# anzeA/Tarok

Measured on AMD Instinct MI355X. Metric: env steps/sec at 65 536 parallel 4-player games; 1/2/4/8 MI355X, higher is better.
Workload: dtype u64

## Files before the change

include/tarok_env.h:

```cpp
#ifndef TAROK_ENV_H
#define TAROK_ENV_H
#include <stdint.h>

#ifdef __cplusplus
extern "C" {
#endif

#define TAROK_ABI_VERSION 5
#define TAROK_MAX_CARDS_PER_LAUNCH 192
#define TAROK_GAMES_AHEAD 14

#define TAROK_OK 0
#define TAROK_EINVAL (-1)
#define TAROK_EHIP (-2)
#define TAROK_ENOMEM (-3)
#define TAROK_ENODEV (-4)

#define TAROK_MIX_ALL 0
#define TAROK_MIX_NAVADNA3 1
#define TAROK_MIX_BOT 2
#define TAROK_MIX_FIXED 16

#define TAROK_DEFER_EXCHANGE 1
#define TAROK_AUTO_RESET 2
// ... 7 lines not shown
#define TAROK_OBS_DONE (1ULL << 62)
#define TAROK_OBS_ERROR (1ULL << 63)

#define TAROK_LANE_HAND0 0
#define TAROK_LANE_PILE0 4
#define TAROK_LANE_TALON 8
#define TAROK_LANE_META 9
#define TAROK_NUM_LANES 10

typedef struct tarok_env tarok_env;

const char *tarok_strerror(int code);
int tarok_abi_version(void);
int tarok_device_count(void);
int tarok_last_hip_error(void);

int tarok_create(tarok_env **out, int device, int64_t n_games, uint64_t game_offset,
                 uint64_t seed, int mix, int flags);
void tarok_destroy(tarok_env *env);
int64_t tarok_num_games(const tarok_env *env);

#define TAROK_OPT_REFILL_FAN 2
#define TAROK_OPT_LAZY_REFILL 3
int tarok_set_option(tarok_env *env, int option, int value);

int tarok_reset(tarok_env *env, uint32_t episode, const uint8_t *deals, const int8_t *contract,
                const int8_t *declarer, const int8_t *king_suit, const int8_t *talon_choice,
                const uint8_t *discards, int flags, void *stream);

int tarok_exchange(tarok_env *env, const int8_t *talon_choice, const uint8_t *discards, void *stream);

int tarok_legal_actions(tarok_env *env, uint64_t *obs_out, int8_t *seat_out, void *stream);

int tarok_step(tarok_env *env, const uint8_t *action, int16_t *reward_out, uint8_t *done_out,
               uint16_t *trick_out, uint64_t *obs_out, int flags, void *stream);

int tarok_prefetch(tarok_env *env, void *stream);

int tarok_policy_random(tarok_env *env, const uint64_t *obs, uint8_t *action_out, void *stream);

int tarok_step_random(tarok_env *env, uint8_t *action_out, int16_t *reward_out, uint8_t *done_out,
                      uint16_t *trick_out, uint64_t *obs_out, int flags, void *stream);

int tarok_krog_random(tarok_env *env, int cards, int64_t stride, uint8_t *action_out, int16_t *reward_out,
                      uint8_t *done_out, uint16_t *trick_out, uint64_t *obs_out, int flags, void *stream);

// ... 109 lines not shown
```

tarok_amd/csrc/tarok_env.hip:

```cpp
#include "tarok_device.h"

#include <hip/hip_runtime.h>
#include <stdint.h>
#include <stdio.h>
#include <stdlib.h>
#include <string.h>
#include <type_traits>
#include <utility>

#include "../../include/tarok_env.h"

#define TK_BLOCK 256
#define TK_PF_SLOTS (4 * TK_BLOCK)
#define TK_GRAPH_CACHE 16
#define TK_REFILL_CAP (TK_BLOCK * TK_AHEAD)
#define TK_REFILL_FAN 8
#define TK_RC(group, k) ((((size_t)(group)) * 4 + (k)) * 32)
#define TK_BULK_EVERY 32u
#define TK_BULK_CAP ((TK_BULK_EVERY / 4) * TK_BLOCK)

#define TK_AHEAD TAROK_GAMES_AHEAD
#define TK_LINE(episode) ((u32)(episode) % (u32)TK_AHEAD)
#define TK_FINQ 128
#define TK_STREAM_STORE(ptr, val) __builtin_nontemporal_store((val), (ptr))
#define TK_WAIT_LOADS() __builtin_amdgcn_s_waitcnt(0x0F70)
#define TK_RARE(c) __builtin_expect(!!(c), 0)
#define TK_USUAL(c) __builtin_expect(!!(c), 1)

struct __attribute__((aligned(64))) AuxLine {
    ulonglong2 n01, n23; u64 nkey; u32 nep;
    u32 pad[5];
};
struct __attribute__((aligned(64))) Aux { AuxLine line[TK_AHEAD]; };
static_assert(sizeof(AuxLine) == 64 && sizeof(Aux) == 64 * TK_AHEAD, "64 bytes per next-game line");
static_assert((TK_BLOCK * sizeof(Aux)) % 128 == 0, "a play group's next-game lines end on an L2 line boundary");
static_assert(TK_AHEAD >= 2 && TK_AHEAD <= 15, "epar / cprev are 4-bit fields");
struct __attribute__((aligned(32))) Counters {
    int4 score_sum;
    u32 episode;
    u32 pad[3];
};
static_assert(sizeof(Counters) == 32, "Counters is half a cache line");

struct tarok_env {
    int device;
    int64_t n;
    u64 offset, seed;
    int mix, flags;
    ulonglong2 *s01, *s23;
    Aux *aux;
    Counters *cnt;
    uint16_t *nstale;
    u64 *gkey;
    uint8_t *hist;
    u64 *rlist;
    u32 *rcount;
    u64 *elist;
    u32 *epoch;
    uint32_t refill_fan;
    uint32_t lazy_refill;
    int n_cus;
    float *adam_sumsq;
    u64 *stamps;
    size_t stamps_words;
    int launched;
    hipStream_t cap_stream;
    struct GraphEntry {
        hipGraphExec_t exec;
        int fused, chunk, flags, prefetch;
        void *action, *reward, *done, *obs, *stamps;
        uint32_t fan, lazy;
    } graphs[TK_GRAPH_CACHE];
    int n_graphs;
};

static thread_local int g_last_hip = 0;

#define HIPCHK(x)                                                   \
    do {                                                            \
        hipError_t e_ = (x);                                        \
        if (e_ != hipSuccess) { g_last_hip = (int)e_; return TAROK_EHIP; } \
    } while (0)

static inline dim3 grid_for(int64_t n) { return dim3((unsigned)((n + TK_BLOCK - 1) / TK_BLOCK)); }

__device__ __forceinline__ void load_game(Game &g, const ulonglong2 *s01, const ulonglong2 *s23, int64_t i) {
    ulonglong2 a = s01[i], b = s23[i];
    unpack(g, a.x, a.y, b.x, b.y);
}
__device__ __forceinline__ void store_game(const Game &g, ulonglong2 *s01, ulonglong2 *s23, int64_t i,
                                           bool seats_changed = true) {
    ulonglong2 a;
    pack_play(g, a.x, a.y);
// ... 253 lines not shown
            for (u32 q = 0; q < TK_REFILL_FAN; q++) {
                bool has = q < fan && g0 + q < play_groups;
                cum[q + 1] = cum[q] + (has ? min(tk_ld(&rcount[TK_RC(g0 + q, 2 + which)]), (u32)TK_BULK_CAP) : 0u);
            }
        }
        for (u32 j = tid; j < cum[TK_REFILL_FAN]; j += nthreads) {
            u32 q = 0;
#pragma unroll
            for (u32 r = 1; r < TK_REFILL_FAN; r++) q += j >= cum[r] ? 1u : 0u;
            u32 base = 0;
#pragma unroll
            for (u32 r = 0; r < TK_REFILL_FAN; r++) base = (r == q) ? cum[r] : base;
            u64 en = tk_ld(&lists[((int64_t)(g0 + q) * 2 + which) * cap + (j - base)]);
            deal_into_buffer(aux, (int64_t)(g0 + q) * TK_BLOCK + (u32)(en & 0xFFFF), (u32)(en >> 32), seed, offset, mix);
        }
    }
    if (any || bulk) {
        __syncthreads();
        if (any && tid < fan && g0 + tid < play_groups) rcount[TK_RC(g0 + tid, par ^ 1u)] = 0u;
        if (bulk && tid < fan && g0 + tid < play_groups) rcount[TK_RC(g0 + tid, 2 + which)] = 0u;
    }
}

template <bool HIST>
__device__ __forceinline__ void play_role(
    u32 group, u32 tid,
    int64_t n, u64 seed, u64 offset, int mix, int flags, int cards, int64_t stride, TkCount count, u32 *epoch, u32 play_groups, u32 fan,
    uint8_t *__restrict__ action_out, int16_t *__restrict__ reward,
    uint8_t *__restrict__ done, uint16_t *__restrict__ trick, u64 *__restrict__ obs, uint8_t *__restrict__ hist,
    ulonglong2 *__restrict__ s01, ulonglong2 *__restrict__ s23, Aux *aux, Counters *__restrict__ cnt,
    u64 *__restrict__ gkey, u64 *rlist, u32 *rcount, u64 *__restrict__ stamps) {
    __shared__ unsigned short push_list[TK_REFILL_CAP];
    __shared__ u32 push_ep[TK_BLOCK];
    __shared__ u32 push_count;
    __shared__ u32 finq[TK_BLOCK / 64][9][TK_FINQ];
    __shared__ int sacc[4][TK_BLOCK];
    if (tid == 0) push_count = 0;
    sacc[0][tid] = 0; sacc[1][tid] = 0; sacc[2][tid] = 0; sacc[3][tid] = 0;
    __syncthreads();
    u32 fq_head = 0, fq_n = 0;
    u32 (*fq)[TK_FINQ] = finq[tid >> 6];
    auto drain_finished = [&](u32 cnt_) __attribute__((always_inline)) {
        u32 lane = tid & 63;
        if (lane < cnt_) {
            u32 e = (fq_head + lane) & (TK_FINQ - 1);
            Game f;
            f.A = TK_U64(fq[0][e], fq[1][e]); f.B = TK_U64(fq[2][e], fq[3][e]); f.C = TK_U64(fq[4][e], fq[5][e]);
            u32 m = fq[7][e], ri = fq[8][e];
            f.talon = TK_U64(fq[6][e], (m >> 24) & 15u);
            f.contract = m & 15; f.declarer = (m >> 4) & 3; f.king = (m >> 6) & 3; f.team = (m >> 8) & 15;
            f.tl = (m >> 12) & 7; f.trick_no = (m >> 16) & 15; f.leader = (m >> 20) & 3;
            f.trick = 0; f.nt = 0; f.phase = TK_PHASE_DONE; f.error = 0; f.epar = 0; f.cprev = 0;
            u64 sc = final_scores(f);
            u32 t = ri & 0xFFFFu;
            if (reward) {
                u64 rs = sc;
                if ((flags & TAROK_REWARD_REF) && (f.contract == TK_BERAC || f.contract == TK_ODPRTI_BERAC)) {
                    int dv = f.trick_no >= 12 ? -20 : 20;
                    u32 d = f.declarer;
                    rs = pack_scores(d == 0 ? (int)(int16_t)(sc & 0xFFFF) : dv, d == 1 ? (int)(int16_t)((sc >> 16) & 0xFFFF) : dv,
                                     d == 2 ? (int)(int16_t)((sc >> 32) & 0xFFFF) : dv, d == 3 ? (int)(int16_t)(sc >> 48) : dv);
                }
                reinterpret_cast<u64 *>(reward)[(int64_t)group * TK_BLOCK + t + (int64_t)(ri >> 16) * stride] = rs;
            }
            atomicAdd(&sacc[0][t], (int)(int16_t)(sc & 0xFFFF)); atomicAdd(&sacc[1][t], (int)(int16_t)((sc >> 16) & 0xFFFF));
            atomicAdd(&sacc[2][t], (int)(int16_t)((sc >> 32) & 0xFFFF)); atomicAdd(&sacc[3][t], (int)(int16_t)(sc >> 48));
        }
        fq_head = (fq_head + cnt_) & (TK_FINQ - 1);
        fq_n -= cnt_;
    };
    u64 t_real0 = 0, t_cyc0 = 0, t_play = 0;
    if (stamps) { t_real0 = __builtin_amdgcn_s_memrealtime(); t_cyc0 = __builtin_amdgcn_s_memtime(); }
    int64_t i = (int64_t)group * TK_BLOCK + tid;
    bool valid = i < n;
    int64_t ic = valid ? i : n - 1;
    Game g;
    load_game(g, s01, s23, ic);
    u64 key = gkey[ic];
    bool autoreset = (flags & TAROK_AUTO_RESET) != 0;
    bool berac = g.contract == TK_BERAC || g.contract == TK_ODPRTI_BERAC;
    bool spec = valid && ((g.phase == TK_PHASE_PLAY && (int)g.nt + cards >= 4 &&
                           (berac || (int)(g.trick_no * 4 + g.nt) + cards >= 48)) ||
                          g.phase == TK_PHASE_DONE);
    u32 cprev0 = valid ? g.cprev : 0u;
    u32 allowed = TK_AHEAD - min(cprev0, (u32)TK_AHEAD);
    int4 acc = make_int4(0, 0, 0, 0);
    u32 cur_ep = 0;
    ulonglong2 na = make_ulonglong2(0, 0), nb = na, na2 = na, nb2 = na;
    u64 nkey = 0, nkey2 = 0;
    u32 nep1 = 0, nep2 = 0;
    bool ok1 = false, ok2 = false;
    auto line_tag = [&](bool &ok, u32 &nep, u32 tag) __attribute__((always_inline)) { nep = tag; ok = true; };
// ... 22 lines not shown
    u64 legal = (valid && g.phase == TK_PHASE_PLAY) ? legal_now(g) : 0;
    u64 c_lead = 0;
    u64 pending = 0;
    u32 blocked_v = 0, resync_v = 0;
    auto fetch_lines = [&](bool lacks, bool lacks2) __attribute__((always_inline)) {
        if (lacks) {
            const AuxLine *ln = &aux[i].line[TK_LINE(cur_ep + 1)];
            na = ln->n01; nb = ln->n23; nkey = ln->nkey;
            line_tag(ok1, nep1, ln->nep);
        }
        if (lacks2) {
            const AuxLine *l2 = &aux[i].line[TK_LINE(cur_ep + 2)];
            na2 = l2->n01; nb2 = l2->n23; nkey2 = l2->nkey;
            line_tag(ok2, nep2, l2->nep);
        }
    };
    auto play_card = [&](auto all_tag, auto nt_tag, auto std_tag, int64_t row, int ci) __attribute__((always_inline)) {
        constexpr bool ALL = decltype(all_tag)::value;
        constexpr int NT = decltype(nt_tag)::value;
        constexpr bool STD = decltype(std_tag)::value;
        if constexpr (NT >= 0) g.nt = (u32)NT;
        constexpr bool TOP_UP_EARLY = ALL && NT == 0;
        constexpr bool TOP_UP_LATE = !(ALL && NT == 3);
        if constexpr (TOP_UP_EARLY) {
            if (TK_RARE(pending != 0)) {
                pending = 0;
                bool base = spec && blocked_v == 0 && consumed >= 1;
                bool lacks = base && nep1 != cur_ep + 1 && consumed < allowed;
                bool lacks2 = base && nep2 != cur_ep + 2 && consumed + 1 < allowed;
                fetch_lines(lacks, lacks2);
            }
        }
        const bool v = ALL ? true : valid;
        const bool play = ALL ? true : (valid && g.phase == TK_PHASE_PLAY);
        u32 a = play ? policy_action(key, g.trick_no * 4 + g.nt, legal) : 255u;
        u64 scores = 0;
        u32 trick_info = 0;
        int res = -2;
        const u32 pos = g.trick_no * 4 + g.nt;
        if constexpr (ALL && NT == 0) c_lead = g.C;
        const u64 *lead_plane = (ALL && NT >= 0) ? &c_lead : nullptr;
        if (play) res = apply_step<true, true>(g, a, scores, trick_info, !STD && trick != nullptr, lead_plane);
        bool fin = res == 1;
        if (HIST && hist && play && res >= 0) hist[(int64_t)pos * n + i] = (uint8_t)a;
        if constexpr (!(ALL && NT >= 0)) {
            touched = touched || res != -2;
            seats_dirty = seats_dirty || (res >= 0 && g.nt == 0);
        }
        if (v) {
            if (STD || action_out) TK_STREAM_STORE(&action_out[row], (uint8_t)a);
            if (!STD && trick) TK_STREAM_STORE(&trick[row], (uint16_t)trick_info);
        }
        constexpr bool CAN_END = !(ALL && NT >= 0 && NT < 3);
        constexpr bool FAST_RENEW = ALL && NT == 3;
        auto push_finished = [&](u64 fm, u32 slot0) __attribute__((always_inline)) {
            u32 e = (slot0 + __builtin_amdgcn_mbcnt_hi((u32)(fm >> 32), __builtin_amdgcn_mbcnt_lo((u32)fm, 0))) & (TK_FINQ - 1);
            fq[0][e] = TK_LO(g.A); fq[1][e] = TK_HI(g.A); fq[2][e] = TK_LO(g.B); fq[3][e] = TK_HI(g.B);
            fq[4][e] = TK_LO(g.C); fq[5][e] = TK_HI(g.C); fq[6][e] = TK_LO(g.talon);
            u32 m = (g.declarer << 4) | g.contract;      TK_KEEP_VGPR(m);
            m = (g.king << 6) | m;                       TK_KEEP_VGPR(m);
            m = (g.team << 8) | m;                       TK_KEEP_VGPR(m);
            m = (g.tl << 12) | m;                        TK_KEEP_VGPR(m);
            m = (g.trick_no << 16) | m;                  TK_KEEP_VGPR(m);
            m = (g.leader << 20) | m;                    TK_KEEP_VGPR(m);
            fq[7][e] = (TK_HI(g.talon) << 24) | m;
            fq[8][e] = ((u32)ci << 16) | tid;
        };
        auto swap_in = [&]() __attribute__((always_inline)) {
            unpack_fresh(g, na.x, na.y, nb.x, nb.y);
            key = nkey;
            na = na2; nb = nb2; nkey = nkey2;
            nep1 = nep2;
        };
        auto deal_in_place = [&](bool deal_here, Game &gd, u64 &kd) __attribute__((always_inline)) {
            u64 pend = __ballot(deal_here);
            if (TK_RARE(pend != 0)) {
                u64 dkey = 0;
                if (deal_here) dkey = game_key(seed, offset + (u64)i, cur_ep + 1);
                u64 h0 = 0, h1 = 0, h2 = 0, h3 = 0, tal = 0;
                u32 lane = __lane_id();
                while (pend) {
                    int l = __builtin_ctzll(pend);
                    pend &= pend - 1;
                    u32 klo = (u32)__builtin_amdgcn_readlane((int)(u32)dkey, l);
                    u32 khi = (u32)__builtin_amdgcn_readlane((int)(u32)(dkey >> 32), l);
                    u64 w0, w1, w2, w3, wt;
                    deal_wave(klo, khi, w0, w1, w2, w3, wt);
                    if (lane == (u32)l) { h0 = w0; h1 = w1; h2 = w2; h3 = w3; tal = wt; }
                }
                if (deal_here) {
                    u32 cc, d, k;
                    sample_setup(dkey, mix, cc, d, k);
                    setup_game(gd, h0, h1, h2, h3, tal, cc, d, k);
                    gd.epar = TK_LINE(cur_ep + 1); gd.cprev = 0;
                    if (gd.phase == TK_PHASE_EXCHANGE) bot_exchange(gd, dkey);
                    kd = dkey;
                }
            }
        };
        if constexpr (FAST_RENEW) {
            u64 fm = __ballot(fin);
            if (TK_USUAL(fm != 0)) {
                if (TK_RARE(fq_n >= 64)) drain_finished(64);
                const u32 slot0 = fq_head + fq_n;
                fq_n += (u32)__popcll(fm);
                if (TK_RARE((fm & __ballot(nep1 != cur_ep + 1)) != 0)) {
                    bool lineless = fin && nep1 != cur_ep + 1;
                    resync_v |= (lineless && consumed < allowed) ? 1u : 0u;
                    blocked_v |= lineless ? 1u : 0u;
                    Game d = g;
                    u64 dk = key;
                    deal_in_place(lineless, d, dk);
                    if (lineless) { pack(d, na.x, na.y, nb.x, nb.y); nkey = dk; nep1 = cur_ep + 1; }
                }
                pending |= fm & __ballot(nep2 != cur_ep + 2);
                if (fin) { push_finished(fm, slot0); swap_in(); cur_ep++; consumed++; }
            }
        }
        if constexpr (CAN_END && !FAST_RENEW) {
            u64 fm = __ballot(fin);
            if (TK_USUAL(fm != 0)) {
                if (TK_RARE(fq_n >= 64)) drain_finished(64);
                if (fin) push_finished(fm, fq_head + fq_n);
                fq_n += (u32)__popcll(fm);
            }
        }
        if (CAN_END && !FAST_RENEW && (ALL || autoreset)) {
            bool renew = ALL ? fin : (v && g.phase == TK_PHASE_DONE);
            if (TK_USUAL(__ballot(renew) != 0)) {
                if constexpr (TOP_UP_LATE) {
                    bool lacks = spec && !blocked && !ok1 && consumed >= 1 && consumed < allowed;
                    if (TK_RARE(__ballot(renew && lacks) != 0)) {
                        bool lacks2 = spec && !blocked && !ok2 && consumed >= 1 && consumed + 1 < allowed;
                        fetch_lines(lacks, lacks2);
                        TK_WAIT_LOADS();
                    }
                }
                bool swap = renew && !blocked && ok1 && nep1 == cur_ep + 1;
                if (swap) {
                    swap_in();
                    ok1 = ok2 && consumed + 1 < allowed;
                    ok2 = false;
                }
                bool deal_here = renew && !swap;
                if (deal_here && consumed < allowed) resync = true;
// ... 11 lines not shown
    };
    int64_t row = i;
    typedef std::integral_constant<int, -1> nt_any;
    if (autoreset && __ballot(valid && g.phase == TK_PHASE_PLAY) == ~0ULL) {
        if ((cards & 3) == 0 && __ballot(g.nt != 0) == 0) {
            auto tricks = [&](auto std_tag) __attribute__((always_inline)) {
                touched = true; seats_dirty = true;
                for (int c = 0; c < cards; c += 4) {
                    play_card(std::true_type{}, std::integral_constant<int, 0>{}, std_tag, row, c); row += stride;
                    play_card(std::true_type{}, std::integral_constant<int, 1>{}, std_tag, row, c + 1); row += stride;
                    play_card(std::true_type{}, std::integral_constant<int, 2>{}, std_tag, row, c + 2); row += stride;
                    play_card(std::true_type{}, std::integral_constant<int, 3>{}, std_tag, row, c + 3); row += stride;
                }
            };
            if (action_out && done && !trick) tricks(std::true_type{});
            else tricks(std::false_type{});
        } else {
            for (int c = 0; c < cards; c++, row += stride) play_card(std::true_type{}, nt_any{}, std::false_type{}, row, c);
        }
    } else {
        for (int c = 0; c < cards; c++, row += stride) play_card(std::false_type{}, nt_any{}, std::false_type{}, row, c);
    }
    while (fq_n) drain_finished(min(fq_n, 64u));
    __builtin_amdgcn_s_waitcnt(0xC07F);
    {
        int4 sa = make_int4(sacc[0][tid], sacc[1][tid], sacc[2][tid], sacc[3][tid]);
        if (sa.x | sa.y | sa.z | sa.w) { acc.x += sa.x; acc.y += sa.y; acc.z += sa.z; acc.w += sa.w; acc_dirty = true; }
    }
    u32 np = (resync || resync_v != 0) ? (u32)TK_AHEAD : min(consumed, (u32)TK_AHEAD);
    if (valid) {
        g.cprev = np;
        if (acc_dirty) cnt[i].score_sum = acc;
        if (consumed) { cnt[i].episode = cur_ep; gkey[i] = key; }
        if (touched || consumed || cprev0 != np) store_game(g, s01, s23, i, seats_dirty || cprev0 != np);
    }
    if (stamps) t_play = __builtin_amdgcn_s_memtime() - t_cyc0;
    if (valid && np) {
        u32 pos = atomicAdd(&push_count, np);
        push_ep[tid] = cur_ep;
        for (u32 j = 0; j < np; j++) push_list[pos + j] = (unsigned short)(j * TK_BLOCK + tid);
    }
    __syncthreads();
    u32 total = push_count;
    u64 *lst = rlist + ((int64_t)group * 2 + par) * TK_REFILL_CAP;
    for (u32 j = tid; j < total; j += TK_BLOCK) {
        u32 en = push_list[j], t = en % TK_BLOCK;
        lst[j] = ((u64)(push_ep[t] + TK_AHEAD - en / TK_BLOCK) << 32) | t;
    }
    if (tid == 0) rcount[TK_RC(group, par)] = total;
    if (stamps && (tid & 63) == 0) {
        u64 w = (u64)i >> 6;
        stamps[3 * w + 0] = t_real0;
        stamps[3 * w + 1] = __builtin_amdgcn_s_memrealtime();
        stamps[3 * w + 2] = ((__builtin_amdgcn_s_memtime() - t_cyc0) << 32) | (t_play & 0xFFFFFFFFULL);
    }
}

#define TK_PLAY_ARGS                                                                                                             \
    int64_t n, u64 seed, u64 offset, int mix, int flags, int cards, int64_t stride, u32 play_groups, u32 *epoch, u32 fan,         \
        uint8_t *__restrict__ action_out, int16_t *__restrict__ reward,                                                           \
        uint8_t *__restrict__ done, uint16_t *__restrict__ trick, u64 *__restrict__ obs, uint8_t *__restrict__ hist,              \
        ulonglong2 *__restrict__ s01, ulonglong2 *__restrict__ s23, Aux *aux, Counters *__restrict__ cnt,                         \
        u64 *__restrict__ gkey, u64 *rlist, u32 *rcount, u64 *__restrict__ stamps
template <bool HIST>
TK_KERNEL(TK_BLOCK, 168) __attribute__((amdgpu_waves_per_eu(3, 3))) void k_play_wide(TK_PLAY_ARGS) {
    TK_VGPR_TOP(168, 167);
    TkCount count = launch_count<1>(epoch, play_groups);
    if (blockIdx.x >= play_groups)
        refill_role<false>(blockIdx.x - play_groups, threadIdx.x, TK_BLOCK, seed, offset, mix, play_groups, count, epoch, fan, false, aux, rlist, rcount, nullptr);
    else {
        play_role<HIST>(blockIdx.x, threadIdx.x, n, seed, offset, mix, flags, cards, stride, count, epoch, play_groups, fan,
                        action_out, reward, done, trick, obs, hist, s01, s23, aux, cnt, gkey, rlist, rcount, stamps);
    }
}

__device__ __forceinline__ void deal_in_place_wave(bool deal_here, Game &gd, u64 &kd, u64 seed, u64 offset, int64_t i, u32 ep, int mix) {
    u64 pend = __ballot(deal_here);
    if (pend == 0) return;
    u64 dkey = 0;
    if (deal_here) dkey = game_key(seed, offset + (u64)i, ep);
    u64 h0 = 0, h1 = 0, h2 = 0, h3 = 0, tal = 0;
    u32 lane = __lane_id();
    while (pend) {
        int l = __builtin_ctzll(pend);
        pend &= pend - 1;
        u32 klo = (u32)__builtin_amdgcn_readlane((int)(u32)dkey, l);
        u32 khi = (u32)__builtin_amdgcn_readlane((int)(u32)(dkey >> 32), l);
        u64 w0, w1, w2, w3, wt;
        deal_wave(klo, khi, w0, w1, w2, w3, wt);
        if (lane == (u32)l) { h0 = w0; h1 = w1; h2 = w2; h3 = w3; tal = wt; }
    }
    if (deal_here) {
        u32 cc, d, k;
        sample_setup(dkey, mix, cc, d, k);
// ... 1404 lines not shown
        default: return "unknown error";
    }
}

int tarok_abi_version(void) { return TAROK_ABI_VERSION; }
int tarok_last_hip_error(void) { return g_last_hip; }

int tarok_device_count(void) {
    int n = 0;
    if (hipGetDeviceCount(&n) != hipSuccess) { (void)hipGetLastError(); return 0; }
    return n;
}

int tarok_create(tarok_env **out, int device, int64_t n_games, uint64_t game_offset, uint64_t seed, int mix, int flags) {
    if (!out || n_games <= 0 || n_games > (1LL << 31) || (flags & ~TAROK_HISTORY)) return TAROK_EINVAL;
    if (!(mix == TAROK_MIX_ALL || mix == TAROK_MIX_NAVADNA3 || mix == TAROK_MIX_BOT || (mix >= TAROK_MIX_FIXED && mix < TAROK_MIX_FIXED + 10))) return TAROK_EINVAL;
    if (device < 0 || device >= tarok_device_count()) return TAROK_ENODEV;
    HIPCHK(hipSetDevice(device));
    tarok_env *e = new tarok_env();
    memset(e, 0, sizeof *e);
    e->device = device; e->n = n_games; e->offset = game_offset; e->seed = seed; e->mix = mix; e->flags = flags;
    e->refill_fan = n_games >= (1 << 20) ? TK_REFILL_FAN : (n_games >= (1 << 18) ? 4 : 1);
    e->lazy_refill = n_games < (1 << 20) ? 1 : 0;
    size_t stale_bytes = (size_t)((n_games + TK_PF_SLOTS - 1) / TK_PF_SLOTS) * TK_PF_SLOTS * sizeof(uint16_t);
    hipError_t r = hipMalloc((void **)&e->s01, (size_t)n_games * sizeof(ulonglong2));
    if (r == hipSuccess) r = hipMalloc((void **)&e->s23, (size_t)n_games * sizeof(ulonglong2));
    if (r == hipSuccess) r = hipMalloc((void **)&e->aux, (size_t)n_games * sizeof(Aux));
    if (r == hipSuccess) r = hipMalloc((void **)&e->cnt, (size_t)n_games * sizeof(Counters));
    if (r == hipSuccess) r = hipMalloc((void **)&e->nstale, stale_bytes);
    if (r == hipSuccess) r = hipMalloc((void **)&e->gkey, (size_t)n_games * sizeof(u64));
    if (r == hipSuccess && (flags & TAROK_HISTORY)) r = hipMalloc((void **)&e->hist, (size_t)n_games * 48);
    if (r == hipSuccess && e->hist) r = hipMemset(e->hist, 255, (size_t)n_games * 48);
    size_t groups = (size_t)((n_games + TK_BLOCK - 1) / TK_BLOCK);
    if (r == hipSuccess) r = hipMalloc((void **)&e->rlist, groups * 2 * TK_REFILL_CAP * sizeof(u64));
    if (r == hipSuccess) r = hipMalloc((void **)&e->rcount, TK_RC(groups, 0) * sizeof(u32));
    if (r == hipSuccess) r = hipMalloc((void **)&e->elist, groups * 2 * TK_BULK_CAP * sizeof(u64));
    if (r == hipSuccess) r = hipMalloc((void **)&e->adam_sumsq, 1024 * sizeof(float));
    if (r == hipSuccess) r = hipMalloc((void **)&e->epoch, 2 * TK_EPOCH_WORDS * sizeof(u32));
    if (r == hipSuccess) r = hipMemset(e->epoch, 0, 2 * TK_EPOCH_WORDS * sizeof(u32));
    if (r == hipSuccess) r = hipMemset(e->rcount, 0, TK_RC(groups, 0) * sizeof(u32));
    if (r == hipSuccess) r = hipMemset(e->s01, 0, (size_t)n_games * sizeof(ulonglong2));
    if (r == hipSuccess) r = hipMemset(e->s23, 0, (size_t)n_games * sizeof(ulonglong2));
    if (r == hipSuccess) r = hipMemset(e->aux, 0, (size_t)n_games * sizeof(Aux));
    if (r == hipSuccess) r = hipMemset(e->cnt, 0, (size_t)n_games * sizeof(Counters));
    if (r == hipSuccess) r = hipMemset(e->nstale, 0, stale_bytes);
    if (r == hipSuccess) r = hipMemset(e->gkey, 0, (size_t)n_games * sizeof(u64));
// ... 17 lines not shown
    if (!e) return;
    (void)hipSetDevice(e->device);
    drop_graphs(e);
    if (e->cap_stream) (void)hipStreamDestroy(e->cap_stream);
    (void)hipFree(e->s01); (void)hipFree(e->s23); (void)hipFree(e->aux); (void)hipFree(e->cnt); (void)hipFree(e->nstale); (void)hipFree(e->gkey);
    (void)hipFree(e->rlist); (void)hipFree(e->rcount); (void)hipFree(e->elist); (void)hipFree(e->epoch); (void)hipFree(e->hist); (void)hipFree(e->adam_sumsq);
    delete e;
}

int64_t tarok_num_games(const tarok_env *e) { return e ? e->n : 0; }

int tarok_set_option(tarok_env *e, int option, int value) {
    if (!e) return TAROK_EINVAL;
    if (option == TAROK_OPT_REFILL_FAN && value >= 1 && value <= TK_REFILL_FAN) {
        if ((uint32_t)value != e->refill_fan && e->launched) {
            HIPCHK(hipSetDevice(e->device));
            HIPCHK(hipDeviceSynchronize());
            HIPCHK(hipMemset(e->epoch, 0, 2 * TK_EPOCH_WORDS * sizeof(u32)));
            HIPCHK(hipMemset(e->rcount, 0, TK_RC((e->n + TK_BLOCK - 1) / TK_BLOCK, 0) * sizeof(u32)));
        }
        e->refill_fan = (uint32_t)value;
    } else if (option == TAROK_OPT_LAZY_REFILL && (value == 0 || value == 1)) {
        e->lazy_refill = (uint32_t)value;
    } else return TAROK_EINVAL;
    return TAROK_OK;
}

static inline void launch_prefetch(tarok_env *e, hipStream_t s) {
    dim3 grid((unsigned)((e->n + TK_PF_SLOTS - 1) / TK_PF_SLOTS));
    hipLaunchKernelGGL(k_prefetch, grid, dim3(TK_BLOCK), 0, s, e->n, e->seed, e->offset, e->mix, e->aux, e->cnt, e->nstale);
}

int tarok_reset(tarok_env *e, uint32_t episode, const uint8_t *deals, const int8_t *contract, const int8_t *declarer,
                const int8_t *king_suit, const int8_t *talon_choice, const uint8_t *discards, int flags, void *stream) {
    if (!e) return TAROK_EINVAL;
    if ((talon_choice == nullptr) != (discards == nullptr)) return TAROK_EINVAL;
    if (contract && !declarer) return TAROK_EINVAL;
    HIPCHK(hipSetDevice(e->device));
    HIPCHK(hipMemsetAsync(e->rcount, 0, TK_RC((e->n + TK_BLOCK - 1) / TK_BLOCK, 0) * sizeof(u32), (hipStream_t)stream));
    hipLaunchKernelGGL(k_reset, grid_for(e->n), dim3(TK_BLOCK), 0, (hipStream_t)stream, e->n, e->seed, e->offset,
                       episode, e->mix, flags, deals, contract, declarer, king_suit, talon_choice, discards, e->s01,
                       e->s23, e->aux, e->cnt, e->nstale, e->gkey);
    launch_prefetch(e, (hipStream_t)stream);
    HIPCHK(hipGetLastError());
    return TAROK_OK;
}
// ... 24 lines not shown
    return TAROK_OK;
}

static inline u64 *stamps_for(const tarok_env *e, size_t words) { return (e->stamps && e->stamps_words >= words) ? e->stamps : nullptr; }

static inline void launch_play(tarok_env *e, bool random, int cards, int64_t stride, const uint8_t *action_in,
                               uint8_t *action_out, int16_t *reward, uint8_t *done, uint16_t *trick, uint64_t *obs,
                               int flags, hipStream_t s) {
    u32 groups = (u32)((e->n + TK_BLOCK - 1) / TK_BLOCK);
    u32 fan = e->refill_fan;
    dim3 grid(groups + (groups + fan - 1) / fan);
    e->launched = 1;
    if (cards == 1 && e->lazy_refill) grid = dim3(groups);
    if (cards == 1) {
#define TK_LAUNCH_STEP(R, Z)                                                                                             \
    hipLaunchKernelGGL((k_step<R, Z>), grid, dim3(TK_BLOCK), 0, s, e->n, e->seed, e->offset, e->mix, flags, groups, e->epoch, \
                       fan, action_in, action_out, reward, done, trick, (u64 *)obs, e->hist, e->s01, e->s23, e->aux, e->cnt,  \
                       e->gkey, e->rlist, e->rcount, e->elist)
        if (e->lazy_refill) { if (random) TK_LAUNCH_STEP(true, true); else TK_LAUNCH_STEP(false, true); }
        else                { if (random) TK_LAUNCH_STEP(true, false); else TK_LAUNCH_STEP(false, false); }
#undef TK_LAUNCH_STEP
        return;
    }
#define TK_LAUNCH_PLAY(H)                                                                                              \
    hipLaunchKernelGGL((k_play_wide<H>), grid, dim3(TK_BLOCK), 0, s, e->n, e->seed, e->offset, e->mix, flags, cards, stride, \
                       groups, e->epoch, fan, action_out, reward, done, trick, (u64 *)obs, e->hist, e->s01,            \
                       e->s23, e->aux, e->cnt, e->gkey, e->rlist, e->rcount, stamps)
    u64 *stamps = stamps_for(e, 3 * (size_t)((e->n + 63) / 64));
    if (e->hist) TK_LAUNCH_PLAY(true); else TK_LAUNCH_PLAY(false);
#undef TK_LAUNCH_PLAY
}

int tarok_step(tarok_env *e, const uint8_t *action, int16_t *reward_out, uint8_t *done_out, uint16_t *trick_out,
               uint64_t *obs_out, int flags, void *stream) {
    if (!e || !action || !obs_out) return TAROK_EINVAL;
    HIPCHK(hipSetDevice(e->device));
    launch_play(e, false, 1, e->n, action, nullptr, reward_out, done_out, trick_out, obs_out, flags, (hipStream_t)stream);
    HIPCHK(hipGetLastError());
    return TAROK_OK;
}

static inline void launch_policy(tarok_env *e, const uint64_t *obs, uint8_t *action, hipStream_t s) {
    if (e->n >= (1 << 21) && (((uintptr_t)obs & 15) | ((uintptr_t)action & 1)) == 0)
        hipLaunchKernelGGL(k_policy_x4, dim3((unsigned)((e->n + 4 * TK_BLOCK - 1) / (4 * TK_BLOCK))), dim3(TK_BLOCK), 0, s, e->n,
                           (const u64 *)obs, e->gkey, action);
    else
        hipLaunchKernelGGL(k_policy, grid_for(e->n), dim3(TK_BLOCK), 0, s, e->n, (const u64 *)obs, e->gkey, action);
}

int tarok_policy_random(tarok_env *e, const uint64_t *obs, uint8_t *action_out, void *stream) {
    if (!e || !obs || !action_out) return TAROK_EINVAL;
    HIPCHK(hipSetDevice(e->device));
// ... 29 lines not shown
        launch_policy(e, obs, action, s);
        launch_play(e, false, 1, e->n, action, nullptr, reward, done, nullptr, obs, flags, s);
    }
}

int tarok_run_random(tarok_env *e, int64_t n_steps, int cards_per_launch, int graph_chunk, int prefetch_every,
                     uint8_t *action, int16_t *reward_out, uint8_t *done_out, uint64_t *obs_out, int flags, void *stream) {
    if (!e || !obs_out || n_steps < 0 || graph_chunk < 0 || graph_chunk > 8192 || prefetch_every < 0) return TAROK_EINVAL;
    if (cards_per_launch < 0 || cards_per_launch > TAROK_MAX_CARDS_PER_LAUNCH) return TAROK_EINVAL;
    int unit = cards_per_launch >= 2 ? cards_per_launch : 1;
    if (n_steps % unit != 0 || graph_chunk % unit != 0) return TAROK_EINVAL;
    if (prefetch_every % unit != 0) return TAROK_EINVAL;
    if (graph_chunk > 0 && prefetch_every > 0 && graph_chunk % prefetch_every != 0) return TAROK_EINVAL;
    if (!(flags & TAROK_AUTO_RESET)) prefetch_every = 0;
    if (cards_per_launch == 0 && !action) return TAROK_EINVAL;
    HIPCHK(hipSetDevice(e->device));
    hipStream_t s = (hipStream_t)stream;
    int64_t left = n_steps;
    if (graph_chunk > 0 && left >= graph_chunk) {
        hipGraphExec_t gexec = nullptr;
        for (int k = 0; k < e->n_graphs && !gexec; k++) {
            const tarok_env::GraphEntry &g = e->graphs[k];
            if (g.fused == cards_per_launch && g.chunk == graph_chunk && g.flags == flags && g.prefetch == prefetch_every &&
                g.action == action && g.reward == reward_out && g.done == done_out && g.obs == obs_out && g.stamps == e->stamps &&
                g.fan == e->refill_fan && g.lazy == e->lazy_refill)
                gexec = g.exec;
        }
        if (!gexec) {
            if (e->n_graphs == TK_GRAPH_CACHE) drop_graphs(e);
            hipGraph_t graph = nullptr;
            HIPCHK(hipStreamBeginCapture(e->cap_stream, hipStreamCaptureModeRelaxed));
            for (int k = 0; k < graph_chunk; k += unit) {
                launch_one(e, cards_per_launch, action, reward_out, done_out, obs_out, flags, e->cap_stream);
                if (prefetch_every && (k + unit) % prefetch_every == 0) launch_prefetch(e, e->cap_stream);
            }
            HIPCHK(hipStreamEndCapture(e->cap_stream, &graph));
            hipError_t r = hipGraphInstantiate(&gexec, graph, nullptr, nullptr, 0);
            (void)hipGraphDestroy(graph);
            if (r != hipSuccess) { g_last_hip = (int)r; return TAROK_EHIP; }
            e->graphs[e->n_graphs++] = {gexec, cards_per_launch, graph_chunk, flags, prefetch_every, action, reward_out, done_out,
                                        obs_out, e->stamps, e->refill_fan, e->lazy_refill};
        }
        while (left >= graph_chunk) {
            HIPCHK(hipGraphLaunch(gexec, s));
            left -= graph_chunk;
        }
    }
    for (int64_t k = 0; left > 0; left -= unit, k += unit) {
        launch_one(e, cards_per_launch, action, reward_out, done_out, obs_out, flags, s);
        if (prefetch_every && (k + unit) % prefetch_every == 0) launch_prefetch(e, s);
    }
    HIPCHK(hipGetLastError());
    return TAROK_OK;
}

int tarok_rollout_random(tarok_env *e, uint32_t episode, int16_t *scores_out, int16_t *nsteps_out, int8_t *seats_out,
                         uint64_t *masks_out, uint8_t *actions_out, void *stream) {
    if (!e) return TAROK_EINVAL;
    HIPCHK(hipSetDevice(e->device));
    hipLaunchKernelGGL(k_rollout, grid_for(e->n), dim3(TK_BLOCK), 0, (hipStream_t)stream, e->n, e->seed, e->offset,
                       episode, e->mix, scores_out, nsteps_out, seats_out, (u64 *)masks_out, actions_out);
    HIPCHK(hipGetLastError());
    return TAROK_OK;
}
// ... 238 lines not shown
                      float *running, void *stream) {
    if (!e || B < 1 || !feature_words || !rec || !stats || !w1 || !b1 || !w2 || !b2 || !w3 || !b3 || !w3t || !w2t || !Xw || !H1 || !H2 ||
        !dOut || !dH2 || !dH1 || !scratch || !terms_out)
        return TAROK_EINVAL;
    HIPCHK(hipSetDevice(e->device));
    LearnArgs a;
    a.B = B; a.words = (const u64 *)feature_words; a.index = index; a.rec = (const float4 *)rec; a.stats = (const float4 *)stats;
    a.clip = clip; a.vf_coef = vf_coef; a.ent_coef = ent_coef;
    a.w1 = (const __bf16 *)w1; a.w2 = (const __bf16 *)w2; a.w3 = (const __bf16 *)w3; a.w3t = (const __bf16 *)w3t; a.w2t = (const __bf16 *)w2t;
    a.b1 = b1; a.b2 = b2; a.b3 = b3;
    a.Xw = (ulonglong2 *)Xw;
    a.H1 = (uint4 *)H1; a.H2 = (uint4 *)H2; a.dH2 = (uint4 *)dH2; a.dH1 = (uint4 *)dH1; a.dOut = (uint2 *)dOut;
    a.part = (float4 *)scratch;
    unsigned blocks = (unsigned)((B + LN_M - 1) / LN_M);
    a.stamps = stamps_for(e, 8 * (size_t)blocks);
    hipLaunchKernelGGL(k_learn_chain, dim3(blocks), dim3(LN_CHAIN_THREADS), 0, (hipStream_t)stream, a);
    hipLaunchKernelGGL(k_learn_terms, dim3(1), dim3(TK_BLOCK), 0, (hipStream_t)stream, (int)blocks, (const float4 *)scratch,
                       (float4 *)terms_out, (float4 *)running);
    HIPCHK(hipGetLastError());
    return TAROK_OK;
}

static inline void learn_chunks(tarok_env *e, u32 &c2, u32 &c1, u32 &c3) {
    if (!e->n_cus) {
        hipDeviceProp_t pr;
        e->n_cus = hipGetDeviceProperties(&pr, e->device) == hipSuccess && pr.multiProcessorCount > 0 ? pr.multiProcessorCount : 256;
    }
    u32 total = (u32)e->n_cus < 8 ? 8 : (u32)e->n_cus;
    c2 = total * 96 / 256; c1 = total * 108 / 256; c3 = total - c2 - c1;
}

int64_t tarok_learn_workspace_bytes(tarok_env *e) {
    if (!e) return 0;
    u32 c2, c1, c3;
    learn_chunks(e, c2, c1, c3);
    return (int64_t)sizeof(float) * ((int64_t)(c2 + c1) * 65792 + (int64_t)c3 * 16448);
}

int tarok_learn_dw(tarok_env *e, int64_t B, const uint64_t *Xw, const void *H1, const void *H2,
                   const void *dOut, const void *dH2, const void *dH1, const float *terms, void *workspace, float *grad_out,
                   void *stream) {
    if (!e || B < 1 || !Xw || !H1 || !H2 || !dOut || !dH2 || !dH1 || !terms || !workspace || !grad_out) return TAROK_EINVAL;
    if (B > TAROK_LEARN_MAX_BATCH) return TAROK_EINVAL;
    HIPCHK(hipSetDevice(e->device));
    u32 c2, c1, c3;
    learn_chunks(e, c2, c1, c3);
    hipLaunchKernelGGL(k_learn_dw, dim3(c2 + c1 + c3), dim3(TK_BLOCK), 0, (hipStream_t)stream, B, c2, c1, c3, (const u64 *)Xw,
                       (const uint4 *)H1, (const uint4 *)H2, (const uint4 *)dOut, (const uint4 *)dH2, (const uint4 *)dH1,
                       (float *)workspace);
    hipLaunchKernelGGL(k_learn_reduce, dim3((LN_P + TK_BLOCK - 1) / TK_BLOCK), dim3(TK_BLOCK), 0, (hipStream_t)stream, c2, c1, c3,
// ... 51 lines not shown
```

tarok_amd/env.py:

```python
import ctypes as C

import numpy as np
import torch

from . import _native
from . import karte as K


def _u64(t):
    return t.detach().cpu().numpy().view(np.uint64)


class Obs:

    def __init__(self, words):
        self.words = words

    @property
    def mask(self):
        return self.words & K.OBS_MASK

    @property
    def seat(self):
        return (self.words >> K.OBS_SEAT_SHIFT) & 3

    @property
    def step(self):
        return (self.words >> K.OBS_STEP_SHIFT) & 63

    @property
    def done(self):
        return ((self.words >> K.OBS_DONE_BIT) & 1).bool()

    @property
    def error(self):
        return self.words < 0

    def mask_numpy(self):
        return _u64(self.mask)


class TarokVecEnv:
    def __init__(self, n_games, device=0, seed=0, mix=K.MIX_ALL, game_offset=0, history=False, refill_fan=None, lazy_refill=None):
        self._h = None
        L = _native.lib()
        if not torch.cuda.is_available() or L.tarok_device_count() == 0:
            raise _native.TarokNativeError("TarokVecEnv needs an MI355X: no GPU is visible and there is no CPU fallback")
        self.L = L
        self.n = int(n_games)
        self.device_index = int(device)
        self.device = torch.device("cuda", self.device_index)
        self.seed, self.mix, self.game_offset = int(seed), int(mix), int(game_offset)
        h = C.c_void_p()
        self.history = bool(history)
        _native.check(L.tarok_create(C.byref(h), self.device_index, self.n, self.game_offset, self.seed, self.mix,
                                     K.HISTORY if history else 0))
        self._h = h
        self.set_option(refill_fan, lazy_refill)
        with torch.cuda.device(self.device):
            self.obs_words = torch.zeros(self.n, dtype=torch.int64, device=self.device)
            self.reward = torch.zeros((self.n, 4), dtype=torch.int16, device=self.device)
            self.done = torch.zeros(self.n, dtype=torch.uint8, device=self.device)
            self.action = torch.full((self.n,), 255, dtype=torch.uint8, device=self.device)
            self.trick = None

    def set_option(self, refill_fan=None, lazy_refill=None):
        if refill_fan is not None:
            _native.check(self.L.tarok_set_option(self._h, K.OPT_REFILL_FAN, int(refill_fan)))
        if lazy_refill is not None:
            _native.check(self.L.tarok_set_option(self._h, K.OPT_LAZY_REFILL, int(lazy_refill)))

    def refill_selftest(self, kind, per_slot, episode0=100, order=0, reps=1):
        import numpy as np
        rep = np.zeros(49, np.uint64)
        with torch.cuda.device(self.device):
            torch.cuda.synchronize(self.device)
            _native.check(self.L.tarok_debug_refill_selftest(self._h, int(kind), int(per_slot), int(episode0), int(order), int(reps),
                                                             rep.ctypes.data))
        return int(rep[0]), rep[1:].reshape(8, 6)[: min(8, int(rep[0]))]

    def close(self):
        if self._h is not None:
            torch.cuda.synchronize(self.device)
            self.L.tarok_destroy(self._h)
            self._h = None

    def __del__(self):
        try:
            self.close()
        except Exception:
            pass

    def _stream(self):
# ... 352 lines not shown
```

tarok_amd/karte.py:

```python
import enum


class Barva(enum.IntEnum):
    KARA = 0
    SRCE = 1
    PIK = 2
    KRIZ = 3
    TAROK = 4


class Tip(enum.IntEnum):
    Klop = 0
    Tri = 1
    Dve = 2
    Ena = 3
    Solo_tri = 4
    Solo_dve = 5
    Solo_ena = 6
    Berac = 7
    Solo_brez = 8
    Odprti_berac = 9


DECK = (1 << 54) - 1
PAGAT, MOND, SKIS = 32, 52, 53

MIX_ALL = 0
MIX_NAVADNA3 = 1
MIX_BOT = 2
MIX_FIXED = 16

DEFER_EXCHANGE = 1
AUTO_RESET = 2
CLEAR_COUNTERS = 4
REWARD_REF = 8
HISTORY = 16
OPT_REFILL_FAN = 2
OPT_LAZY_REFILL = 3
GAMES_AHEAD = 14
MLP_W1, MLP_B1, MLP_W2, MLP_B2, MLP_W3, MLP_B3, MLP_PARAMS = 0, 65536, 65792, 131328, 131584, 147968, 148032
LEARN_PAD = 256
LEARN_MAX_BATCH = 4194048

REF_ROWS = 56
REF_OPP, REF_OWN, REF_TALON, REF_KING, REF_INDEX, REF_DISCARDS, REF_LEGAL = 0, 9072, 12096, 12426, 12430, 12434, 12488
REF_RECORD_BYTES = 12544
REF_EXCHANGE_BYTES = 400
REF_TYPES = ("Klop", "Navadna_igra", "Solo", "Berac")

OBS_MASK = DECK
OBS_SEAT_SHIFT = 54
OBS_STEP_SHIFT = 56
OBS_DONE_BIT = 62
OBS_ERROR_BIT = 63

PHASE_EXCHANGE, PHASE_PLAY, PHASE_DONE = 1, 2, 3


def card_id(barva, st):
    return 32 + st - 1 if int(barva) == 4 else int(barva) * 8 + st - 1

# ... 21 lines not shown
```

Before: 186.7 billion.

## Add dedicated scorer wave that scores finished games from shared-memory rings

Each play block gets an extra 64-thread wave. Play waves hand batches of 64 finished games to it through per-wave rings in LDS, which are doubled to 256 entries, and the scorer wave computes their scores concurrently. When the scorer falls two batches behind, a play wave scores the batch inline instead. The goal is to take end-of-game scoring off the play waves' critical path, at the cost of more LDS, an extra spinning wave per CU, and new cross-wave handshakes through volatile counters. The scorer path is enabled by default when the number of play groups does not exceed the CU count, and a new option can turn it off.

```diff
diff --git a/include/tarok_env.h b/include/tarok_env.h
--- a/include/tarok_env.h
+++ b/include/tarok_env.h
@@ -53,6 +53,7 @@
 
 #define TAROK_OPT_REFILL_FAN 2
 #define TAROK_OPT_LAZY_REFILL 3
+#define TAROK_OPT_SCORER_WAVE 4
 int tarok_set_option(tarok_env *env, int option, int value);
 
 int tarok_reset(tarok_env *env, uint32_t episode, const uint8_t *deals, const int8_t *contract,
diff --git a/tarok_amd/csrc/tarok_env.hip b/tarok_amd/csrc/tarok_env.hip
--- a/tarok_amd/csrc/tarok_env.hip
+++ b/tarok_amd/csrc/tarok_env.hip
@@ -21,7 +21,9 @@
 
 #define TK_AHEAD TAROK_GAMES_AHEAD
 #define TK_LINE(episode) ((u32)(episode) % (u32)TK_AHEAD)
-#define TK_FINQ 128
+#define TK_FINQ 256
+#define TK_FINQ_INLINE 128
+#define TK_DIAG_DRAINS (1 << 30)
 #define TK_STREAM_STORE(ptr, val) __builtin_nontemporal_store((val), (ptr))
 #define TK_WAIT_LOADS() __builtin_amdgcn_s_waitcnt(0x0F70)
 #define TK_RARE(c) __builtin_expect(!!(c), 0)
@@ -60,6 +62,7 @@
     uint32_t refill_fan;
     uint32_t lazy_refill;
     int n_cus;
+    uint32_t scorer_wave;
     float *adam_sumsq;
     u64 *stamps;
     size_t stamps_words;
@@ -69,6 +72,7 @@
         hipGraphExec_t exec;
         int fused, chunk, flags, prefetch;
         void *action, *reward, *done, *obs, *stamps;
+        size_t stamps_words;
         uint32_t fan, lazy;
     } graphs[TK_GRAPH_CACHE];
     int n_graphs;
@@ -368,7 +372,7 @@
     }
 }
 
-template <bool HIST>
+template <bool HIST, bool SCORER>
 __device__ __forceinline__ void play_role(
     u32 group, u32 tid,
     int64_t n, u64 seed, u64 offset, int mix, int flags, int cards, int64_t stride, TkCount count, u32 *epoch, u32 play_groups, u32 fan,
@@ -379,17 +383,25 @@
     __shared__ unsigned short push_list[TK_REFILL_CAP];
     __shared__ u32 push_ep[TK_BLOCK];
     __shared__ u32 push_count;
-    __shared__ u32 finq[TK_BLOCK / 64][9][TK_FINQ];
+    constexpr u32 FINQ = SCORER ? TK_FINQ : TK_FINQ_INLINE;
+    __shared__ u32 finq[TK_BLOCK / 64][9][FINQ];
     __shared__ int sacc[4][TK_BLOCK];
+    __shared__ u32 handed[SCORER ? TK_BLOCK / 64 : 1], scored[SCORER ? TK_BLOCK / 64 : 1], play_done;
     if (tid == 0) push_count = 0;
-    sacc[0][tid] = 0; sacc[1][tid] = 0; sacc[2][tid] = 0; sacc[3][tid] = 0;
+    if constexpr (SCORER) {
+        if (tid < TK_BLOCK / 64) { handed[tid] = 0; scored[tid] = 0; }
+        if (tid == 0) play_done = 0;
+    }
+    if (!SCORER || tid < TK_BLOCK) { sacc[0][tid] = 0; sacc[1][tid] = 0; sacc[2][tid] = 0; sacc[3][tid] = 0; }
     __syncthreads();
     u32 fq_head = 0, fq_n = 0;
-    u32 (*fq)[TK_FINQ] = finq[tid >> 6];
-    auto drain_finished = [&](u32 cnt_) __attribute__((always_inline)) {
+    u32 (*fq)[FINQ] = finq[SCORER ? (tid >> 6) & 3 : tid >> 6];
+    auto score_batch = [&](u32 (*ring)[FINQ], u32 head, u32 cnt_) __attribute__((always_inline)) {
+        u32 (*fq)[FINQ] = ring;
+        u32 fq_head = head;
         u32 lane = tid & 63;
         if (lane < cnt_) {
-            u32 e = (fq_head + lane) & (TK_FINQ - 1);
+            u32 e = (fq_head + lane) & (FINQ - 1);
             Game f;
             f.A = TK_U64(fq[0][e], fq[1][e]); f.B = TK_U64(fq[2][e], fq[3][e]); f.C = TK_U64(fq[4][e], fq[5][e]);
             u32 m = fq[7][e], ri = fq[8][e];
@@ -412,8 +424,52 @@
             atomicAdd(&sacc[0][t], (int)(int16_t)(sc & 0xFFFF)); atomicAdd(&sacc[1][t], (int)(int16_t)((sc >> 16) & 0xFFFF));
             atomicAdd(&sacc[2][t], (int)(int16_t)((sc >> 32) & 0xFFFF)); atomicAdd(&sacc[3][t], (int)(int16_t)(sc >> 48));
         }
-        fq_head = (fq_head + cnt_) & (TK_FINQ - 1);
+    };
+    auto drain_finished = [&](u32 cnt_) __attribute__((always_inline)) {
+        score_batch(fq, fq_head, cnt_);
+        fq_head = (fq_head + cnt_) & (FINQ - 1);
         fq_n -= cnt_;
+    };
+    if constexpr (SCORER) {
+        if (tid >= TK_BLOCK) {
+            u32 nscored[TK_BLOCK / 64] = {0, 0, 0, 0};
+            for (;;) {
+                u32 pd = (u32)__builtin_amdgcn_readfirstlane((int)*(volatile u32 *)&play_done);
+                bool any = false;
+#pragma unroll
+                for (u32 w = 0; w < TK_BLOCK / 64; w++) {
+                    u32 h = (u32)__builtin_amdgcn_readfirstlane((int)*(volatile u32 *)&handed[w]);
+                    while (nscored[w] != h) {
+                        asm volatile("" ::: "memory");
+                        score_batch(finq[w], (nscored[w] * 64u) & (FINQ - 1), 64);
+                        nscored[w]++;
+                        asm volatile("" ::: "memory");
+                        *(volatile u32 *)&scored[w] = nscored[w];
+                        any = true;
+                    }
+                }
+                if (pd == TK_BLOCK / 64) break;
+                if (!any) __builtin_amdgcn_s_sleep(8);
+            }
+            __syncthreads();
+            return;
+        }
+    }
+    u32 nhanded = 0, scored_seen = 0;
+    u32 inline_drains = 0;
+    auto make_room = [&](u32 seen) __attribute__((always_inline)) {
+        if constexpr (SCORER) {
+            if (TK_USUAL(nhanded - seen < 2u)) {
+                nhanded++;
+                asm volatile("" ::: "memory");
+                *(volatile u32 *)&handed[(tid >> 6) & 3] = nhanded;
+                fq_head = (fq_head + 64u) & (FINQ - 1);
+            } else {
+                score_batch(fq, fq_head + fq_n - 64u, 64);
+                inline_drains++;
+            }
+            fq_n -= 64u;
+        } else drain_finished(64);
     };
     u64 t_real0 = 0, t_cyc0 = 0, t_play = 0;
     if (stamps) { t_real0 = __builtin_amdgcn_s_memrealtime(); t_cyc0 = __builtin_amdgcn_s_memtime(); }
@@ -482,6 +538,7 @@
         if constexpr (NT >= 0) g.nt = (u32)NT;
         constexpr bool TOP_UP_EARLY = ALL && NT == 0;
         constexpr bool TOP_UP_LATE = !(ALL && NT == 3);
+        if constexpr (SCORER && TOP_UP_EARLY) scored_seen = *(volatile u32 *)&scored[(tid >> 6) & 3];
         if constexpr (TOP_UP_EARLY) {
             if (TK_RARE(pending != 0)) {
                 pending = 0;
@@ -514,7 +571,7 @@
         constexpr bool CAN_END = !(ALL && NT >= 0 && NT < 3);
         constexpr bool FAST_RENEW = ALL && NT == 3;
         auto push_finished = [&](u64 fm, u32 slot0) __attribute__((always_inline)) {
-            u32 e = (slot0 + __builtin_amdgcn_mbcnt_hi((u32)(fm >> 32), __builtin_amdgcn_mbcnt_lo((u32)fm, 0))) & (TK_FINQ - 1);
+            u32 e = (slot0 + __builtin_amdgcn_mbcnt_hi((u32)(fm >> 32), __builtin_amdgcn_mbcnt_lo((u32)fm, 0))) & (FINQ - 1);
             fq[0][e] = TK_LO(g.A); fq[1][e] = TK_HI(g.A); fq[2][e] = TK_LO(g.B); fq[3][e] = TK_HI(g.B);
             fq[4][e] = TK_LO(g.C); fq[5][e] = TK_HI(g.C); fq[6][e] = TK_LO(g.talon);
             u32 m = (g.declarer << 4) | g.contract;      TK_KEEP_VGPR(m);
@@ -561,7 +618,10 @@
         if constexpr (FAST_RENEW) {
             u64 fm = __ballot(fin);
             if (TK_USUAL(fm != 0)) {
-                if (TK_RARE(fq_n >= 64)) drain_finished(64);
+                if (TK_RARE(fq_n >= 64)) {
+                    if constexpr (SCORER) make_room((u32)__builtin_amdgcn_readfirstlane((int)scored_seen));
+                    else drain_finished(64);
+                }
                 const u32 slot0 = fq_head + fq_n;
                 fq_n += (u32)__popcll(fm);
                 if (TK_RARE((fm & __ballot(nep1 != cur_ep + 1)) != 0)) {
@@ -580,7 +640,10 @@
         if constexpr (CAN_END && !FAST_RENEW) {
             u64 fm = __ballot(fin);
             if (TK_USUAL(fm != 0)) {
-                if (TK_RARE(fq_n >= 64)) drain_finished(64);
+                if (TK_RARE(fq_n >= 64)) {
+                    if constexpr (SCORER) make_room((u32)__builtin_amdgcn_readfirstlane((int)*(volatile u32 *)&scored[(tid >> 6) & 3]));
+                    else drain_finished(64);
+                }
                 if (fin) push_finished(fm, fq_head + fq_n);
                 fq_n += (u32)__popcll(fm);
             }
@@ -638,8 +701,11 @@
         for (int c = 0; c < cards; c++, row += stride) play_card(std::false_type{}, nt_any{}, std::false_type{}, row, c);
     }
     while (fq_n) drain_finished(min(fq_n, 64u));
-    __builtin_amdgcn_s_waitcnt(0xC07F);
-    {
+    if constexpr (SCORER) {
+        asm volatile("" ::: "memory");
+        if ((tid & 63) == 0) atomicAdd(&play_done, 1u);
+    } else {
+        __builtin_amdgcn_s_waitcnt(0xC07F);
         int4 sa = make_int4(sacc[0][tid], sacc[1][tid], sacc[2][tid], sacc[3][tid]);
         if (sa.x | sa.y | sa.z | sa.w) { acc.x += sa.x; acc.y += sa.y; acc.z += sa.z; acc.w += sa.w; acc_dirty = true; }
     }
@@ -657,6 +723,10 @@
         for (u32 j = 0; j < np; j++) push_list[pos + j] = (unsigned short)(j * TK_BLOCK + tid);
     }
     __syncthreads();
+    if constexpr (SCORER) {
+        int4 sa = make_int4(sacc[0][tid], sacc[1][tid], sacc[2][tid], sacc[3][tid]);
+        if (valid && (sa.x | sa.y | sa.z | sa.w)) cnt[i].score_sum = make_int4(acc.x + sa.x, acc.y + sa.y, acc.z + sa.z, acc.w + sa.w);
+    }
     u32 total = push_count;
     u64 *lst = rlist + ((int64_t)group * 2 + par) * TK_REFILL_CAP;
     for (u32 j = tid; j < total; j += TK_BLOCK) {
@@ -666,6 +736,7 @@
     if (tid == 0) rcount[TK_RC(group, par)] = total;
     if (stamps && (tid & 63) == 0) {
         u64 w = (u64)i >> 6;
+        if (SCORER && (flags & TK_DIAG_DRAINS)) stamps[3 * (u64)((n + 63) >> 6) + w] = ((u64)nhanded << 32) | inline_drains;
         stamps[3 * w + 0] = t_real0;
         stamps[3 * w + 1] = __builtin_amdgcn_s_memrealtime();
         stamps[3 * w + 2] = ((__builtin_amdgcn_s_memtime() - t_cyc0) << 32) | (t_play & 0xFFFFFFFFULL);
@@ -678,14 +749,16 @@
         uint8_t *__restrict__ done, uint16_t *__restrict__ trick, u64 *__restrict__ obs, uint8_t *__restrict__ hist,              \
         ulonglong2 *__restrict__ s01, ulonglong2 *__restrict__ s23, Aux *aux, Counters *__restrict__ cnt,                         \
         u64 *__restrict__ gkey, u64 *rlist, u32 *rcount, u64 *__restrict__ stamps
-template <bool HIST>
-TK_KERNEL(TK_BLOCK, 168) __attribute__((amdgpu_waves_per_eu(3, 3))) void k_play_wide(TK_PLAY_ARGS) {
+#define TK_PLAY_THREADS(SCORER) ((SCORER) ? TK_BLOCK + 64 : TK_BLOCK)
+template <bool HIST, bool SCORER>
+TK_KERNEL(TK_PLAY_THREADS(SCORER), 168) __attribute__((amdgpu_waves_per_eu(3, 3))) void k_play_wide(TK_PLAY_ARGS) {
     TK_VGPR_TOP(168, 167);
     TkCount count = launch_count<1>(epoch, play_groups);
-    if (blockIdx.x >= play_groups)
+    if (blockIdx.x >= play_groups) {
+        if (SCORER && threadIdx.x >= TK_BLOCK) return;
         refill_role<false>(blockIdx.x - play_groups, threadIdx.x, TK_BLOCK, seed, offset, mix, play_groups, count, epoch, fan, false, aux, rlist, rcount, nullptr);
-    else {
-        play_role<HIST>(blockIdx.x, threadIdx.x, n, seed, offset, mix, flags, cards, stride, count, epoch, play_groups, fan,
+    } else {
+        play_role<HIST, SCORER>(blockIdx.x, threadIdx.x, n, seed, offset, mix, flags, cards, stride, count, epoch, play_groups, fan,
                         action_out, reward, done, trick, obs, hist, s01, s23, aux, cnt, gkey, rlist, rcount, stamps);
     }
 }
@@ -2136,6 +2209,11 @@
     e->device = device; e->n = n_games; e->offset = game_offset; e->seed = seed; e->mix = mix; e->flags = flags;
     e->refill_fan = n_games >= (1 << 20) ? TK_REFILL_FAN : (n_games >= (1 << 18) ? 4 : 1);
     e->lazy_refill = n_games < (1 << 20) ? 1 : 0;
+    e->scorer_wave = 1;
+    {
+        hipDeviceProp_t pr;
+        e->n_cus = hipGetDeviceProperties(&pr, device) == hipSuccess && pr.multiProcessorCount > 0 ? pr.multiProcessorCount : 256;
+    }
     size_t stale_bytes = (size_t)((n_games + TK_PF_SLOTS - 1) / TK_PF_SLOTS) * TK_PF_SLOTS * sizeof(uint16_t);
     hipError_t r = hipMalloc((void **)&e->s01, (size_t)n_games * sizeof(ulonglong2));
     if (r == hipSuccess) r = hipMalloc((void **)&e->s23, (size_t)n_games * sizeof(ulonglong2));
@@ -2199,6 +2277,12 @@
         e->refill_fan = (uint32_t)value;
     } else if (option == TAROK_OPT_LAZY_REFILL && (value == 0 || value == 1)) {
         e->lazy_refill = (uint32_t)value;
+    } else if (option == TAROK_OPT_SCORER_WAVE && (value == 0 || value == 1)) {
+        if ((uint32_t)value != e->scorer_wave) {
+            HIPCHK(hipSetDevice(e->device));
+            drop_graphs(e);
+        }
+        e->scorer_wave = (uint32_t)value;
     } else return TAROK_EINVAL;
     return TAROK_OK;
 }
@@ -2269,12 +2353,16 @@
 #undef TK_LAUNCH_STEP
         return;
     }
-#define TK_LAUNCH_PLAY(H)                                                                                              \
-    hipLaunchKernelGGL((k_play_wide<H>), grid, dim3(TK_BLOCK), 0, s, e->n, e->seed, e->offset, e->mix, flags, cards, stride, \
-                       groups, e->epoch, fan, action_out, reward, done, trick, (u64 *)obs, e->hist, e->s01,            \
+#define TK_LAUNCH_PLAY(H, S)                                                                                                     \
+    hipLaunchKernelGGL((k_play_wide<H, S>), grid, dim3(TK_PLAY_THREADS(S)), 0, s, e->n, e->seed, e->offset, e->mix, flags, cards, \
+                       stride, groups, e->epoch, fan, action_out, reward, done, trick, (u64 *)obs, e->hist, e->s01,                \
                        e->s23, e->aux, e->cnt, e->gkey, e->rlist, e->rcount, stamps)
-    u64 *stamps = stamps_for(e, 3 * (size_t)((e->n + 63) / 64));
-    if (e->hist) TK_LAUNCH_PLAY(true); else TK_LAUNCH_PLAY(false);
+    size_t waves = (size_t)((e->n + 63) / 64);
+    u64 *stamps = stamps_for(e, 3 * waves);
+    if (stamps && e->stamps_words >= 4 * waves) flags |= TK_DIAG_DRAINS;
+    const bool scorer = e->scorer_wave && groups <= (u32)e->n_cus;
+    if (scorer) { if (e->hist) TK_LAUNCH_PLAY(true, true); else TK_LAUNCH_PLAY(false, true); }
+    else        { if (e->hist) TK_LAUNCH_PLAY(true, false); else TK_LAUNCH_PLAY(false, false); }
 #undef TK_LAUNCH_PLAY
 }
 
@@ -2350,7 +2438,7 @@
         for (int k = 0; k < e->n_graphs && !gexec; k++) {
             const tarok_env::GraphEntry &g = e->graphs[k];
             if (g.fused == cards_per_launch && g.chunk == graph_chunk && g.flags == flags && g.prefetch == prefetch_every &&
-                g.action == action && g.reward == reward_out && g.done == done_out && g.obs == obs_out && g.stamps == e->stamps &&
+                g.action == action && g.reward == reward_out && g.done == done_out && g.obs == obs_out && g.stamps == e->stamps && g.stamps_words == e->stamps_words &&
                 g.fan == e->refill_fan && g.lazy == e->lazy_refill)
                 gexec = g.exec;
         }
@@ -2367,7 +2455,7 @@
             (void)hipGraphDestroy(graph);
             if (r != hipSuccess) { g_last_hip = (int)r; return TAROK_EHIP; }
             e->graphs[e->n_graphs++] = {gexec, cards_per_launch, graph_chunk, flags, prefetch_every, action, reward_out, done_out,
-                                        obs_out, e->stamps, e->refill_fan, e->lazy_refill};
+                                        obs_out, e->stamps, e->stamps_words, e->refill_fan, e->lazy_refill};
         }
         while (left >= graph_chunk) {
             HIPCHK(hipGraphLaunch(gexec, s));
@@ -2652,10 +2740,6 @@
 }
 
 static inline void learn_chunks(tarok_env *e, u32 &c2, u32 &c1, u32 &c3) {
-    if (!e->n_cus) {
-        hipDeviceProp_t pr;
-        e->n_cus = hipGetDeviceProperties(&pr, e->device) == hipSuccess && pr.multiProcessorCount > 0 ? pr.multiProcessorCount : 256;
-    }
     u32 total = (u32)e->n_cus < 8 ? 8 : (u32)e->n_cus;
     c2 = total * 96 / 256; c1 = total * 108 / 256; c3 = total - c2 - c1;
 }
diff --git a/tarok_amd/env.py b/tarok_amd/env.py
--- a/tarok_amd/env.py
+++ b/tarok_amd/env.py
@@ -41,7 +41,8 @@
 
 
 class TarokVecEnv:
-    def __init__(self, n_games, device=0, seed=0, mix=K.MIX_ALL, game_offset=0, history=False, refill_fan=None, lazy_refill=None):
+    def __init__(self, n_games, device=0, seed=0, mix=K.MIX_ALL, game_offset=0, history=False, refill_fan=None, lazy_refill=None,
+                 scorer_wave=None):
         self._h = None
         L = _native.lib()
         if not torch.cuda.is_available() or L.tarok_device_count() == 0:
@@ -56,7 +57,7 @@
         _native.check(L.tarok_create(C.byref(h), self.device_index, self.n, self.game_offset, self.seed, self.mix,
                                      K.HISTORY if history else 0))
         self._h = h
-        self.set_option(refill_fan, lazy_refill)
+        self.set_option(refill_fan, lazy_refill, scorer_wave)
         with torch.cuda.device(self.device):
             self.obs_words = torch.zeros(self.n, dtype=torch.int64, device=self.device)
             self.reward = torch.zeros((self.n, 4), dtype=torch.int16, device=self.device)
@@ -64,11 +65,13 @@
             self.action = torch.full((self.n,), 255, dtype=torch.uint8, device=self.device)
             self.trick = None
 
-    def set_option(self, refill_fan=None, lazy_refill=None):
+    def set_option(self, refill_fan=None, lazy_refill=None, scorer_wave=None):
         if refill_fan is not None:
             _native.check(self.L.tarok_set_option(self._h, K.OPT_REFILL_FAN, int(refill_fan)))
         if lazy_refill is not None:
             _native.check(self.L.tarok_set_option(self._h, K.OPT_LAZY_REFILL, int(lazy_refill)))
+        if scorer_wave is not None:
+            _native.check(self.L.tarok_set_option(self._h, K.OPT_SCORER_WAVE, int(scorer_wave)))
 
     def refill_selftest(self, kind, per_slot, episode0=100, order=0, reps=1):
         import numpy as np
diff --git a/tarok_amd/karte.py b/tarok_amd/karte.py
--- a/tarok_amd/karte.py
+++ b/tarok_amd/karte.py
@@ -37,6 +37,7 @@
 HISTORY = 16
 OPT_REFILL_FAN = 2
 OPT_LAZY_REFILL = 3
+OPT_SCORER_WAVE = 4
 GAMES_AHEAD = 14
 MLP_W1, MLP_B1, MLP_W2, MLP_B2, MLP_W3, MLP_B3, MLP_PARAMS = 0, 65536, 65792, 131328, 131584, 147968, 148032
 LEARN_PAD = 256
```

New measurement: 107.4 billion. 42.5% lower.
